# Manta-Network/manta-rs

Measured on AMD Instinct MI355X. Metric: G1 MSM Mscalar/s at 2^20, higher is better.
Workload: dtype u32; 1 GPU; 2^20 BLS12-381 G1 variable-base MSM per GPU, uniform scalars resident in HBM; curve=BLS12-381, log_n=20, window_bits=17, msms_in_flight=3

## Files before the change

### include/mantagpu.h

```cpp
#ifndef MANTAGPU_H
#define MANTAGPU_H
#include <stddef.h>
#include <stdint.h>

#ifdef __cplusplus
extern "C" {
#endif

typedef enum { MG_BN254 = 0, MG_BLS12_381 = 1 } mg_curve_t;

enum {
    MG_SUCCESS = 0,
    MG_ERROR_INVALID_ARGUMENT = 1,
    MG_ERROR_HIP = 2,
    MG_ERROR_OUT_OF_MEMORY = 3,
    MG_ERROR_DOMAIN_TOO_LARGE = 4,
    MG_ERROR_STATE = 5,
    MG_ERROR_CHECKSUM = 6
};

typedef struct mg_bases mg_bases;
typedef struct mg_msm_job mg_msm_job;
typedef struct mg_ctx mg_ctx;

int mg_init(int device);
const char *mg_strerror(int status);
const char *mg_last_error(void);
int mg_device_count(int *count);
int mg_malloc(void **dptr, size_t bytes);
int mg_free(void *dptr);
int mg_memcpy_h2d(void *dptr, const void *hptr, size_t bytes);
int mg_memcpy_d2h(void *hptr, const void *dptr, size_t bytes);
int mg_device_synchronize(void);
int mg_host_alloc(void **hptr, size_t bytes);
int mg_host_free(void *hptr);
int mg_set_kernel_timing(int on);
float mg_last_accumulate_ms(void);
float mg_last_accumulate_mhz(void);
int mg_clock_probe(unsigned iters, double *memtime_mhz, double *mad_issue_per_us_per_simd, double *ms);
int mg_last_ntt_ms(float out4[4]);
int mg_last_prove_phases_ms(float out10[10]);
int mg_last_pass_host_ms(float out3[3]);
int mg_hw_queues(int out2[2]);

int mg_bases_create(mg_curve_t curve, int group, const uint64_t *affine_mont, size_t n, int on_device,
                    int precompute_window_bits, mg_bases **out);
int mg_bases_create_sharded(mg_curve_t curve, int group, const uint64_t *affine_mont, size_t n, const int *devices,
                            int n_devices, int precompute_window_bits, mg_bases **out);
int mg_bases_num_shards(const mg_bases *bases);
int mg_bases_shard(const mg_bases *bases, int shard, int *device, size_t *lo, size_t *hi);
void mg_bases_destroy(mg_bases *bases);
size_t mg_bases_device_bytes(const mg_bases *bases);
int mg_msm(const mg_bases *bases, const uint64_t *scalars_canonical, size_t n, uint64_t *out_affine_mont);
#define MG_SCALARS_MONT 1
#define MG_SCALARS_SPARSE 2
int mg_msm_launch(const mg_bases *bases, const uint64_t *d_scalars, size_t n, int scalar_flags, int window_bits,
                  mg_msm_job **job);
int mg_msm_launch_sharded(const mg_bases *bases, const uint64_t *const *d_scalars_per_shard, int scalar_flags,
                          int window_bits, mg_msm_job **job);
int mg_msm_finish(mg_msm_job *job, uint64_t *out_affine_mont);
int mg_msm_result_to_device(mg_msm_job *job, uint64_t *d_out_xyzz, void *stream);
size_t mg_xyzz_limbs(mg_curve_t curve, int group);
int mg_xyzz_sum(mg_curve_t curve, int group, const uint64_t *xyzz, size_t n, uint64_t *out_affine_mont);
int mg_points_sum(mg_curve_t curve, int group, const uint64_t *affine_mont, size_t n, uint64_t *out_affine_mont);
int mg_fixed_base_mul(mg_curve_t curve, int group, const uint64_t *base_affine_mont, const uint64_t *d_scalars,
                      size_t n, uint64_t *d_out_affine_mont);
#define MG_EC_ADD_MIXED 0
#define MG_EC_ADD 1
#define MG_EC_DOUBLE 2
#define MG_EC_MUL 3
#define MG_EC_SUB_MIXED 4
#define MG_EC_MUL_FIXED 5
int mg_ec_elementwise(mg_curve_t curve, int group, int op, const uint64_t *a_affine, const uint64_t *b, size_t n,
                      uint64_t *out_affine);
#define MG_FIELD_ADD 0
#define MG_FIELD_SUB 1
#define MG_FIELD_MUL 2
#define MG_FIELD_SQR 3
#define MG_FIELD_NEG 4
#define MG_FIELD_FROM_CANONICAL 5
#define MG_FIELD_TO_CANONICAL 6
#define MG_FIELD_INV 7
int mg_field_op(int field, int op, int repr, int lazy_a, int lazy_b, const uint64_t *a, const uint64_t *b, size_t n,
                uint64_t *out);
int mg_msm_digits(mg_curve_t curve, const uint64_t *scalars, size_t batch, size_t n_scalars, int scalar_flags, int window_bits,
                  int table_mode, size_t n, const uint32_t *map, size_t n_sets, size_t set_len, int compact, uint32_t *keys,
                  uint32_t *vals, uint32_t *count, uint32_t layout[4]);
int mg_sort_pairs(const uint32_t *keys, const uint32_t *vals, size_t n, int end_bit, const uint32_t *count, uint32_t lowmask,
                  uint32_t inv_from, uint32_t *keys_out, uint32_t *vals_out);
int mg_group_ntt(mg_curve_t curve, int group, const uint64_t *points_affine, unsigned log_n, int inverse, uint64_t *out_affine);
int mg_point_serialize(mg_curve_t curve, int group, const uint64_t *affine_mont, int compressed, uint8_t *out);

int mg_ntt(mg_curve_t curve, uint64_t *data_mont, unsigned log_n, int inverse, int coset);
int mg_ntt_device(mg_curve_t curve, uint64_t *d_data_mont, unsigned log_n, int inverse, int coset);

typedef struct {
// ... 232 lines not shown
```

### manta_rs_amd/api.py

```python
from __future__ import annotations

import ctypes
import os

import numpy as np

_HERE = os.path.dirname(os.path.abspath(__file__))
LIB_PATH = os.environ.get("MANTA_LIB") or os.path.join(_HERE, "lib", "libmantagpu.so")

BN254, BLS12_381 = 0, 1
FQ_LIMBS = {BN254: 4, BLS12_381: 6}


class MantaGpuError(RuntimeError):

    def __init__(self, status, where=""):
        self.status = status
        detail = LIB.mg_last_error().decode() if status == 2 else ""
        super().__init__(f"{where}: {LIB.mg_strerror(status).decode()} ({status}) {detail}")


def _load():
    if not os.path.exists(LIB_PATH):
        raise ImportError(
            f"{LIB_PATH} not found: the MI355X HIP library is the product and there is no CPU fallback. "
            "Run `python -c 'import __graft_entry__ as g; g.build()'` (or `make -C manta_rs_amd/csrc`).")
    try:
        import torch
    except Exception:
        pass
    lib = ctypes.CDLL(LIB_PATH, mode=ctypes.RTLD_GLOBAL)
    lib.mg_strerror.restype = ctypes.c_char_p
    lib.mg_last_error.restype = ctypes.c_char_p
    lib.mg_bases_device_bytes.restype = ctypes.c_size_t
    lib.mg_ctx_domain_size.restype = ctypes.c_uint64
    lib.mg_ctx_num_variables.restype = ctypes.c_uint64
    lib.mg_ctx_num_inputs.restype = ctypes.c_uint64
    lib.mg_last_accumulate_ms.restype = ctypes.c_float
    lib.mg_last_accumulate_mhz.restype = ctypes.c_float
    lib.mg_vk_encoded_size.restype = ctypes.c_size_t
    lib.mg_vk_num_inputs.restype = ctypes.c_uint64
    lib.mg_xyzz_limbs.restype = ctypes.c_size_t
    lib.mg_partials_slot_limbs.restype = ctypes.c_size_t
    return lib


LIB = _load()
_vp = ctypes.c_void_p
_sz = ctypes.c_size_t

EXPORTS = [
    "mg_init", "mg_strerror", "mg_last_error", "mg_device_count", "mg_malloc", "mg_free", "mg_memcpy_h2d",
    "mg_memcpy_d2h", "mg_device_synchronize", "mg_host_alloc", "mg_host_free", "mg_set_kernel_timing", "mg_last_accumulate_ms", "mg_bases_create", "mg_bases_destroy", "mg_bases_device_bytes",
    "mg_msm", "mg_msm_launch", "mg_msm_finish", "mg_points_sum", "mg_fixed_base_mul", "mg_ec_elementwise", "mg_point_serialize", "mg_ntt",
    "mg_msm_digits", "mg_sort_pairs",
    "mg_ntt_device", "mg_groth16_setup", "mg_ctx_create", "mg_ctx_create_from_bytes", "mg_ctx_set_r1cs", "mg_groth16_prove", "mg_groth16_prove_batch", "mg_witness_map", "mg_ctx_domain_size", "mg_ctx_table_bytes",
    "mg_ctx_destroy", "mg_bases_create_sharded", "mg_bases_num_shards", "mg_bases_shard", "mg_msm_launch_sharded",
    "mg_ctx_create_sharded", "mg_ctx_create_from_bytes_sharded", "mg_ctx_num_variables", "mg_ctx_num_inputs",
    "mg_ctx_num_shards", "mg_field_op", "mg_vk_create", "mg_vk_create_from_bytes", "mg_vk_encoded_size", "mg_vk_encode",
    "mg_vk_alpha_beta", "mg_vk_num_inputs", "mg_vk_destroy", "mg_groth16_verify", "mg_groth16_verify_batch", "mg_pairing_check", "mg_proof_decode", "mg_group_ntt",
    "mg_msm_result_to_device", "mg_xyzz_limbs", "mg_xyzz_sum", "mg_ctx_create_shard", "mg_partials_slot_limbs",
    "mg_groth16_partials_launch", "mg_groth16_partials_finish", "mg_groth16_assemble", "mg_blake3", "mg_ctx_create_from_bytes_checked",
    "mg_last_ntt_ms", "mg_hw_queues", "mg_last_prove_phases_ms", "mg_clock_probe", "mg_last_accumulate_mhz", "mg_ctx_create_task",
    "mg_ctx_opts_init", "mg_ctx_create_ex", "mg_ctx_create_from_bytes_ex", "mg_last_pass_host_ms",
    "mg_tuning_init", "mg_get_tuning", "mg_set_tuning", "mg_tuning_env_names",
    "mg_points_decode", "mg_points_check", "mg_points_encode", "mg_proofs_decode",
    "mg_poseidon_create", "mg_poseidon_destroy", "mg_poseidon_permute", "mg_poseidon_hash", "mg_poseidon_hash_device",
    "mg_merkle_tree", "mg_merkle_forest_roots",
    "mg_edwards_decode", "mg_edwards_encode", "mg_edwards_check", "mg_edwards_mul", "mg_edwards_add",
    "mg_note_cipher_create", "mg_note_cipher_destroy", "mg_notes_encrypt", "mg_notes_decrypt",
    "mg_utxo_model_create", "mg_utxo_model_destroy", "mg_utxos_mint", "mg_utxos_open", "mg_viewing_keys",
    "mg_blake2s256", "mg_schnorr_challenges", "mg_signatures_verify", "mg_signatures_sign",
    "mg_blake2s", "mg_aes256_gcm", "mg_address_partitions", "mg_merkle_shard_indices",
    "mg_light_notes_encrypt", "mg_light_notes_open", "mg_outgoing_notes_encrypt", "mg_outgoing_notes_open",
]


def _chk(rc, where):
    if rc != 0:
        raise MantaGpuError(rc, where)


def _p(a):
    return None if a is None else a.ctypes.data_as(_vp)


def _u64(a):
    return np.ascontiguousarray(a, dtype=np.uint64)


def _addr(x):
    if x is None:
        return None
    if isinstance(x, ctypes.c_void_p):
        return x
    if hasattr(x, "ptr"):
        return _addr(x.ptr)
    return _vp(int(x))


def init(device=0):
    _chk(LIB.mg_init(int(device)), "mg_init")


def device_count():
    c = ctypes.c_int(0)
    _chk(LIB.mg_device_count(ctypes.byref(c)), "mg_device_count")
    return c.value


def set_kernel_timing(on):
    _chk(LIB.mg_set_kernel_timing(int(bool(on))), "mg_set_kernel_timing")


def last_accumulate_ms():
    return float(LIB.mg_last_accumulate_ms())


def last_accumulate_mhz():
    return float(LIB.mg_last_accumulate_mhz())


def clock_probe(iters=200000):
    a, b, c = ctypes.c_double(0), ctypes.c_double(0), ctypes.c_double(0)
    _chk(LIB.mg_clock_probe(ctypes.c_uint(iters), ctypes.byref(a), ctypes.byref(b), ctypes.byref(c)), "mg_clock_probe")
    return a.value, b.value, c.value


def last_ntt_ms():
    v = (ctypes.c_float * 4)()
    _chk(LIB.mg_last_ntt_ms(v), "mg_last_ntt_ms")
    return [float(x) for x in v]


def hw_queues():
    v = (ctypes.c_int * 2)()
    _chk(LIB.mg_hw_queues(v), "mg_hw_queues")
    return int(v[0]), int(v[1])


def last_prove_phases_ms():
    v = (ctypes.c_float * 10)()
    _chk(LIB.mg_last_prove_phases_ms(v), "mg_last_prove_phases_ms")
    names = ("upload_z", "witness_map", "msm_a", "msm_b_g1", "msm_b_g2", "msm_l", "msm_h", "part_a_upload_to_join", "g2_chain_upload_to_end",
             "host_assembly_after_gpu")
    return {n: round(float(x), 4) for n, x in zip(names, v)}


def last_pass_host_ms():
    v = (ctypes.c_float * 3)()
    _chk(LIB.mg_last_pass_host_ms(v), "mg_last_pass_host_ms")
    return {"enqueue": round(float(v[0]), 4), "wait_gpu": round(float(v[1]), 4), "assemble": round(float(v[2]), 4)}


def synchronize():
    _chk(LIB.mg_device_synchronize(), "mg_device_synchronize")


class PinnedArray:

    def __init__(self, shape, dtype=np.uint64):
        self.nbytes = int(np.prod(shape)) * np.dtype(dtype).itemsize
        ptr = _vp()
        _chk(LIB.mg_host_alloc(ctypes.byref(ptr), _sz(self.nbytes)), "mg_host_alloc")
        self._ptr = ptr
        buf = (ctypes.c_uint8 * self.nbytes).from_address(ptr.value)
        self.array = np.frombuffer(buf, dtype=dtype).reshape(shape)

    @classmethod
    def like(cls, arr):
        arr = np.ascontiguousarray(arr)
        p = cls(arr.shape, arr.dtype)
        p.array[...] = arr
        return p

    def free(self):
        if self._ptr is not None and self._ptr.value:
            self.array = None
            LIB.mg_host_free(self._ptr)
            self._ptr = None

    def __del__(self):
        try:
            self.free()
        except Exception:
            pass


class DeviceBuffer:

    def __init__(self, nbytes):
# ... 1099 lines not shown
```

### manta_rs_amd/csrc/capi.cpp

```cpp
#include "../../include/mantagpu.h"
#include "engine.h"
#include "staging.h"
#include "tuning.h"
#include <cstddef>
#include "prover.h"
#include "verify.h"
#include "edwards.h"
#include "utxo.h"
#include "schnorr.h"
#include "light_note.h"
#include <cstring>
#include <new>
#include <vector>

using namespace mg;

struct BasesShard {
    GroupEngine *eng;
    BaseSet *bs;
    int device;
    size_t lo, hi;
};
struct mg_bases {
    std::vector<BasesShard> sh;
// ... 46 lines not shown
    return MG_SUCCESS;
}
MG_API int mg_free(void *dptr) {
    MG_HIP(hipFree(dptr));
    return MG_SUCCESS;
}
MG_API int mg_host_alloc(void **hptr, size_t bytes) {
    if (!hptr) return MG_ERROR_INVALID_ARGUMENT;
    MG_HIP(hipHostMalloc(hptr, bytes ? bytes : 1, hipHostMallocDefault));
    return MG_SUCCESS;
}
MG_API int mg_host_free(void *hptr) {
    MG_HIP(hipHostFree(hptr));
    return MG_SUCCESS;
}
MG_API int mg_memcpy_h2d(void *d, const void *h, size_t bytes) {
    MG_HIP(memcpy_sync(d, h, bytes, hipMemcpyHostToDevice));
    return MG_SUCCESS;
}
MG_API int mg_memcpy_d2h(void *h, const void *d, size_t bytes) {
    MG_HIP(memcpy_sync(h, d, bytes, hipMemcpyDeviceToHost));
    return MG_SUCCESS;
}
MG_API int mg_device_synchronize(void) {
    MG_HIP(hipDeviceSynchronize());
    return MG_SUCCESS;
}

MG_API int mg_set_kernel_timing(int on) {
    set_kernel_timing(on != 0);
    return MG_SUCCESS;
}
MG_API float mg_last_accumulate_ms(void) { return last_accumulate_ms(); }
MG_API float mg_last_accumulate_mhz(void) { return last_accumulate_mhz(); }
namespace mg {
int clock_probe(u32 iters, double *memtime_mhz, double *mad_issue_per_us_per_simd, double *ms);
}
MG_API int mg_clock_probe(unsigned iters, double *memtime_mhz, double *mad_issue_per_us_per_simd, double *ms) {
    MG_TRY
    if (iters == 0 || iters > (1u << 24)) return MG_ERROR_INVALID_ARGUMENT;
    return clock_probe(iters, memtime_mhz, mad_issue_per_us_per_simd, ms);
    MG_CATCH
}
MG_API int mg_last_ntt_ms(float out4[4]) {
    if (!out4) return MG_ERROR_INVALID_ARGUMENT;
    get_last_ntt_ms(out4);
    return MG_SUCCESS;
}
MG_API int mg_hw_queues(int out2[2]) {
    if (!out2) return MG_ERROR_INVALID_ARGUMENT;
    out2[0] = out2[1] = 0;
    (void)stream_queue_counts(&out2[0], &out2[1]);
    return MG_SUCCESS;
}
MG_API int mg_last_pass_host_ms(float out3[3]) {
    if (!out3) return MG_ERROR_INVALID_ARGUMENT;
    get_last_pass_host_ms(out3);
    return MG_SUCCESS;
}
MG_API int mg_last_prove_phases_ms(float out10[10]) {
    if (!out10) return MG_ERROR_INVALID_ARGUMENT;
    get_last_prove_ms(out10);
    return MG_SUCCESS;
}

static void bases_free(mg_bases *b) {
    DeviceGuard guard;
    for (BasesShard &s : b->sh) {
        hipSetDevice(s.device);
        if (s.bs) s.eng->bases_destroy(s.bs);
    }
    delete b;
}
static int bases_create_on(mg_curve_t curve, int group, const uint64_t *affine, size_t n, int on_device, int pre_c,
                           const int *devices, int n_devices, mg_bases **out) {
    if (!out || !affine || n == 0 || pre_c < -12 || pre_c == -1 || pre_c > 24 || n_devices < 1 || n_devices > 64 || (size_t)n_devices > n)
        return MG_ERROR_INVALID_ARGUMENT;
    if (on_device && n_devices != 1) return MG_ERROR_INVALID_ARGUMENT;
    int count = 0;
    MG_HIP(hipGetDeviceCount(&count));
    DeviceGuard guard;
    mg_bases *b = new mg_bases();
    b->n = n;
    for (int g = 0; g < n_devices; ++g) {
        const int dev = devices ? devices[g] : guard.prev;
        if (dev < 0 || dev >= count || dev >= MAX_DEVICES) {
            bases_free(b);
            return MG_ERROR_INVALID_ARGUMENT;
        }
        hipError_t he = hipSetDevice(dev);
        GroupEngine *e = he == hipSuccess ? get_engine((int)curve, group) : nullptr;
        if (!e) {
            bases_free(b);
            return he == hipSuccess ? MG_ERROR_INVALID_ARGUMENT : MG_ERROR_HIP;
        }
        const size_t lo = n * (size_t)g / n_devices, hi = n * (size_t)(g + 1) / n_devices;
        BaseSet *bs = nullptr;
        int rc = e->bases_create((const u32 *)affine + lo * (size_t)e->affine_words(), hi - lo, on_device != 0, pre_c, &bs);
        if (rc) {
            bases_free(b);
            return rc;
        }
        b->sh.push_back(BasesShard{e, bs, dev, lo, hi});
    }
    *out = b;
    return MG_SUCCESS;
// ... 895 lines not shown
```

### manta_rs_amd/csrc/ec_dev.h

```cpp
#pragma once
#include "fp_dev.h"

namespace mg {

#define MG_EC_CALL __device__ __noinline__

template <class F, int B> struct Bv {
    F v;
};
template <int B, class F> MG_DEV Bv<F, B> bv(const F &f) { return Bv<F, B>{f}; }
template <class F, int A, int B> MG_DEV Bv<F, F::BM> operator*(const Bv<F, A> &a, const Bv<F, B> &b) {
    static_assert((long)A * B * F::MULK <= F::LIM, "product of operand bounds exceeds the Montgomery headroom");
    return Bv<F, F::BM>{F::template mulb<A, B>(a.v, b.v)};
}
template <class F, int A> MG_DEV Bv<F, F::BM> b_sqr(const Bv<F, A> &a) {
    static_assert((long)A * A * F::MULK <= F::LIM, "square of operand bound exceeds the Montgomery headroom");
    return Bv<F, F::BM>{F::template sqrb<A>(a.v)};
}
template <class F, int A, int B> MG_DEV Bv<F, A + B> operator+(const Bv<F, A> &a, const Bv<F, B> &b) {
    return Bv<F, A + B>{F::add(a.v, b.v)};
}
template <class F, int A> MG_DEV Bv<F, 2 * A> b_dbl(const Bv<F, A> &a) { return Bv<F, 2 * A>{F::dbl(a.v)}; }
template <class F, int A, int B> MG_DEV Bv<F, A + B> operator-(const Bv<F, A> &a, const Bv<F, B> &b) {
    static_assert(B <= F::MAXM, "no multiple of p large enough for this subtrahend");
// ... 74 lines not shown
        auto X2 = b_sqr(px);
        auto M = b_fit<6>(b_dbl(X2) + X2);
        auto X3 = b_fit<BX>(b_sub2(b_sqr(M), bv<0>(F::zero()), S));
        auto Y3 = b_fit<BY>(M * (S - X3) - W * py);
        X3o = X3.v;
        Y3o = Y3.v;
        Vo = V.v;
        Wo = W.v;
    }
    static MG_EC_CALL XYZZ dbl_affine_call(const Affine<F> &p) { return dbl_affine_body(p); }
    static MG_DEV XYZZ dbl_affine(const Affine<F> &p) {
        if constexpr (F::EXT) return dbl_affine_call(p);
        else return dbl_affine_body(p);
    }
    static MG_DEV XYZZ dbl_affine_body(const Affine<F> &p) {
        XYZZ r;
        dbl_core(bv<BM>(p.x), bv<BM>(p.y), r.x, r.y, r.zz, r.zzz);
        return r;
    }
    static MG_EC_CALL XYZZ dbl_call(const XYZZ &p) { return dbl_body(p); }
    static MG_DEV XYZZ dbl(const XYZZ &p) {
        if constexpr (F::EXT) return dbl_call(p);
        else return dbl_body(p);
    }
    static MG_DEV XYZZ dbl_body(const XYZZ &p) {
        if (p.is_inf()) return p;
        XYZZ r;
        F V, W;
        dbl_core(bv<BX>(p.x), bv<BY>(p.y), r.x, r.y, V, W);
        r.zz = (bv<BM>(V) * bv<BM>(p.zz)).v;
        r.zzz = (bv<BM>(W) * bv<BM>(p.zzz)).v;
        return r;
    }
    MG_EC_CALL void madd_call(const Affine<F> &q, bool neg) { madd_body(q, neg); }
    MG_DEV void madd(const Affine<F> &q, bool neg) {
        if constexpr (F::EXT) madd_call(q, neg);
        else madd_body(q, neg);
    }
#ifdef MG_ACC_TWO_CHAINS
    static constexpr bool THROUGHPUT_CH = false;
#else
    static constexpr bool THROUGHPUT_CH = true;
#endif
    MG_DEV void madd_throughput(const Affine<F> &q, bool neg) {
        if constexpr (!F::EXT && F::LAZY) {
            madd_lazy<THROUGHPUT_CH>(q, neg);
            return;
        }
        madd(q, neg);
    }
    struct MaddCarry {
        F P, R, PP;
    };
    template <bool CH = false> MG_DEV bool madd_begin(const Affine<F> &q_in, bool negate, MaddCarry &c) {
        static_assert(!F::EXT && F::LAZY, "reduced-radix base field only");
        static_assert(F::BX == 8 && F::BY == 4 && F::BM == 2 && F::LIM >= 121, "bound analysis above");
        constexpr bool LL = F::LAZY_LIMBS;
        if (q_in.is_inf()) return false;
        F qy = q_in.y;
        if (negate) {
            if constexpr (LL) qy = F::template negl<3>(q_in.y);
            else qy = F::template neg<2>(q_in.y);
        }
        if (is_inf()) {
            x = q_in.x;
            y = negate ? F::template neg<2>(q_in.y) : q_in.y;
            zz = F::one();
            zzz = F::one();
            return false;
        }
        const F U2 = F::template mul_t<CH>(q_in.x, zz);
        const F S2 = F::template mul_t<CH>(qy, zzz);
        if constexpr (LL) {
            c.P = F::template subl<9>(U2, x);
            c.R = F::template subl<5>(S2, y);
        } else {
            c.P = F::template sub<8>(U2, x);
            c.R = F::template sub<4>(S2, y);
        }
        c.PP = F::template sqr_t<CH>(c.P);
        if (c.PP.template is_zero_mod<2>()) {
            if ((LL ? F::normalize_u(c.R) : c.R).template is_zero_mod<7>()) {
                Affine<F> q{q_in.x, negate ? F::template neg<2>(q_in.y) : q_in.y};
                *this = dbl_affine(q);
            } else {
                *this = inf();
            }
            return false;
        }
        return true;
    }
    template <bool CH = false> MG_DEV void madd_finish(const MaddCarry &c) {
        constexpr bool LL = F::LAZY_LIMBS;
        const F PPP = F::template mul_t<CH>(c.P, c.PP);
        const F Q = F::template mul_t<CH>(x, c.PP);
        const F X3 = F::template sub2<6>(F::template sqr_t<CH>(c.R), PPP, Q);
        F T, N;
        if constexpr (LL) {
            T = F::template subl<9>(Q, X3);
            N = F::template negl<3>(PPP);
        } else {
            T = F::template sub<8>(Q, X3);
            N = F::template neg<2>(PPP);
        }
        const F Y3 = F::template mul_add_t<CH>(c.R, T, y, N);
        zz = F::template mul_t<CH>(zz, c.PP);
        zzz = F::template mul_t<CH>(zzz, PPP);
        x = X3;
        y = Y3;
    }
    template <bool CH = false> MG_DEV void madd_lazy(const Affine<F> &q_in, bool negate) {
        MaddCarry c;
        if (madd_begin<CH>(q_in, negate, c)) madd_finish<CH>(c);
    }
    MG_DEV void madd_body(const Affine<F> &q_in, bool negate) {
        if constexpr (!F::EXT && F::LAZY) {
            madd_lazy<false>(q_in, negate);
            return;
        }
        if (q_in.is_inf()) return;
        Affine<F> q = q_in;
        if (negate) q.y = b_neg(bv<BM>(q.y)).v;
        if (is_inf()) {
            x = q.x;
            y = q.y;
            zz = F::one();
            zzz = F::one();
            return;
        }
        const auto X1 = bv<BX>(x);
        const auto Y1 = bv<BY>(y);
        const auto ZZ1 = bv<BM>(zz);
        const auto ZZZ1 = bv<BM>(zzz);
        auto U2 = bv<BM>(q.x) * ZZ1;
        auto S2 = bv<BM>(q.y) * ZZZ1;
        auto P = U2 - X1;
        auto R = S2 - Y1;
        if (b_is_zero(P)) {
            if (b_is_zero(R))
                *this = dbl_affine(q);
            else
                *this = inf();
            return;
        }
        auto PP = b_sqr(P);
        auto PPP = P * PP;
// ... 103 lines not shown
```

### manta_rs_amd/csrc/engine.h

```cpp
#pragma once
#include <hip/hip_runtime.h>
#include <shared_mutex>
#include <atomic>
#include <cstddef>
#include <cstdint>
#include <mutex>
#include <vector>

namespace mg {

typedef uint32_t u32;
typedef uint64_t u64;

#ifdef MG_NO_PRIO
#define MG_PRIO_HIGH() ((void)0)
#else
#define MG_PRIO_HIGH() __builtin_amdgcn_s_setprio(3)
#endif
#define MG_PRIO_FOR(F) MG_PRIO_HIGH()

enum { MG_OK = 0, MG_ERR_ARG = 1, MG_ERR_HIP = 2, MG_ERR_OOM = 3, MG_ERR_DOMAIN = 4, MG_ERR_STATE = 5 };

void set_last_hip_error(hipError_t e, const char *expr, const char *file, int line);
inline int hip_status(hipError_t e, const char *what, const char *file = __builtin_FILE(), int line = __builtin_LINE()) {
// ... 44 lines not shown
void stream_pool_put_normal(hipStream_t s);
struct GraphClient {
    GraphClient();
    ~GraphClient();
    GraphClient(const GraphClient &) = delete;
    GraphClient &operator=(const GraphClient &) = delete;
};
int graph_clients_alive();
hipStream_t stream_pool_get_dedicated();
void stream_pool_put_dedicated(hipStream_t s);
struct StreamSet {
    hipStream_t main = nullptr, g2 = nullptr, z3 = nullptr;
    int id = -1, dev = 0;
    bool z3_high = false;
};
bool stream_sets_ready();
int stream_queue_counts(int *normal, int *high);
bool stream_set_acquire(StreamSet &s, bool z3_high);
void stream_set_release(StreamSet &s);
int streams_share_queue(hipStream_t a, hipStream_t b, unsigned *mem, unsigned *token_counter);
const char *last_error_string();

struct DeviceScope {
    int prev = 0;
    bool switched = false;
    explicit DeviceScope(int dev) {
        if (hipGetDevice(&prev) == hipSuccess && prev != dev) switched = hipSetDevice(dev) == hipSuccess;
    }
    ~DeviceScope() {
        if (switched) hipSetDevice(prev);
    }
    DeviceScope(const DeviceScope &) = delete;
    DeviceScope &operator=(const DeviceScope &) = delete;
};

struct DeviceGuard {
    int prev = 0;
    DeviceGuard() { hipGetDevice(&prev); }
    ~DeviceGuard() { hipSetDevice(prev); }
    DeviceGuard(const DeviceGuard &) = delete;
    DeviceGuard &operator=(const DeviceGuard &) = delete;
};

struct DevBuf {
    void *p = nullptr;
    size_t cap = 0;
    int reserve(size_t bytes);
    void release();
    template <class T> T *as() const { return (T *)p; }
};

enum { SCALARS_CANONICAL = 0, SCALARS_MONT = 1, SCALARS_WORK = 2 };

struct MsmPlan {
    int c = 0;
    int W = 0;
    u32 B = 0;
    int Wb = 0;
    bool precomp = false;
    bool full = false;
    u32 L = 0;
};

struct BaseSet {
    int curve = 0, group = 1;
    int device = 0;
    size_t n = 0;
    size_t n_orig = 0;
    u32 *d_map = nullptr;
    u32 *d_pts = nullptr;
    int pre_c = 0, pre_W = 0;
    bool full = false;
    u32 n_sets = 1;
    size_t set_len = 0;
    static constexpr u32 MAX_SETS = 4;
    u32 set_first[MAX_SETS + 1] = {};
    size_t bytes = 0;
};

enum MsmTailKind : u32 { TAIL_WINDOW_SUMS = 0, TAIL_X_SUMS = 1, TAIL_TWO_LEVELS = 2 };
struct MsmTail {
    static constexpr int MAX_EXTRA = 8;
    MsmTailKind kind = TAIL_WINDOW_SUMS;
    u32 T1 = 0, nP = 0, segs = 0;
    u32 tail_shift = 0, n_extra = 0, extra_shift[MAX_EXTRA] = {};
    size_t extra_off_pts = 0;
    const u32 *d_tail = nullptr;
};

struct MsmWorkspace {
    DevBuf keys_in, keys_out, vals_in, vals_out, sort_tmp, buckets, pkeys[2], ppts[2], redA, redS, misc;
    DevBuf count;
    DevBuf front, extra;
    DevBuf folded;
    unsigned long long *h_clk = nullptr;
    DevBuf scratch;
    void *h_stage = nullptr;
    size_t h_stage_cap = 0;
    hipStream_t stream = nullptr;
    hipStream_t run_on = nullptr;
    hipStream_t solo = nullptr;
    bool use_solo = false;
    hipStream_t side_stream = nullptr;
    hipEvent_t side_fork = nullptr, side_join = nullptr;
    hipEvent_t done = nullptr;
    hipEvent_t t0 = nullptr, t1 = nullptr;
// ... 110 lines not shown
```

### manta_rs_amd/csrc/msm_accumulate.h

```cpp
#pragma once
#include "msm_common.h"

namespace mg {

#ifndef MG_ACC_INPLACE
#define MG_ACC_INPLACE 1
#endif
#ifndef MG_ACC_BLOCK
#define MG_ACC_BLOCK 0
#endif
#ifndef MG_ACC_AHEAD
#define MG_ACC_AHEAD 0
#endif
#ifndef MG_ACC_SINGLE_ROTATED
#define MG_ACC_SINGLE_ROTATED 0
#endif
template <class F> struct AccChunksRotated : std::false_type {};
template <> struct AccChunksRotated<FpR<Bls381FqCfg>> : std::integral_constant<bool, MG_ACC_INPLACE != 0> {};
template <class F> constexpr bool acc_chunks_rotated() { return AccChunksRotated<F>::value; }
#ifdef MG_ACC_WAVES
#define MG_ACC_ATTR __attribute__((amdgpu_waves_per_eu(MG_ACC_WAVES, MG_ACC_WAVES)))
#else
#define MG_ACC_ATTR
#endif
template <class F, bool PROBE = false>
__global__ __launch_bounds__(256) MG_ACC_ATTR void accumulate_chunks(const u32 *__restrict__ keys, const u32 *__restrict__ vals,
                                                         u32 M, u32 L, u32 invalid, const u32 *__restrict__ bases,
                                                         u32 astride, u32 *__restrict__ buckets,
                                                         u32 *__restrict__ pkeys, u32 *__restrict__ ppts, u32 T,
                                                         const u32 *__restrict__ count, unsigned long long *__restrict__ clk,
                                                         u32 adapt) {
    const u32 t = blockIdx.x * blockDim.x + threadIdx.x;
    if (t >= T) return;
    long long c0 = 0;
    unsigned long long w0 = 0;
    if constexpr (PROBE)
        if (t == 0) c0 = clock64(), w0 = wall_clock64();
    if (count) {
        M = *count;
        if (adapt) {
            const u32 l = (M + T - 1) / T;
            L = l > L ? l : L;
        }
    }
    const size_t begin = (size_t)t * L;
    size_t end = begin + L;
    if (end > M) end = M;
    u32 cur = begin < M ? keys[begin] : invalid;
    if (cur == invalid) {
        pkeys[2 * t] = invalid;
        pkeys[2 * t + 1] = invalid;
        return;
    }
    XYZZ<F> acc = XYZZ<F>::inf();
    bool first = true;
    auto close_run = [&]() {
        if (first) {
            pkeys[2 * t] = cur;
            acc.store(ppts + (size_t)(2 * t) * XYZZ<F>::WORDS);
            first = false;
        } else {
            acc.store(buckets + (size_t)cur * XYZZ<F>::WORDS);
        }
        acc = XYZZ<F>::inf();
    };
    if constexpr (acc_chunks_rotated<F>()) {
        u32 kn = invalid, vn = 0;
        [[maybe_unused]] uint4 kb, vb;
        auto load_block = [&](size_t i) {
            if (i + 4 <= end) {
                kb = *reinterpret_cast<const uint4 *>(keys + i);
                vb = *reinterpret_cast<const uint4 *>(vals + i);
            }
        };
        auto next_pair = [&](size_t i) {
            if constexpr (MG_ACC_BLOCK) {
                const u32 q = (u32)i & 3u;
                if (i - q >= begin && i - q + 4 <= end) {
                    if (q == 0) load_block(i);
                    kn = q == 0 ? kb.x : (q == 1 ? kb.y : (q == 2 ? kb.z : kb.w));
                    vn = q == 0 ? vb.x : (q == 1 ? vb.y : (q == 2 ? vb.z : vb.w));
                    return;
                }
            }
            kn = keys[i], vn = vals[i];
        };
        size_t j = begin;
        u32 k = cur, v = vals[j];
        Affine<F> p = Affine<F>::load(bases + (size_t)(v & 0x7fffffffu) * astride);
        if constexpr (MG_ACC_BLOCK)
            if ((begin & 3) == 0) load_block(begin);
        if (j + 1 < end) next_pair(j + 1);
        bool more;
        do {
            if (k != cur) {
                close_run();
                cur = k;
            }
            typename XYZZ<F>::MaddCarry c;
            const bool general = acc.template madd_begin<XYZZ<F>::THROUGHPUT_CH>(p, (v >> 31) != 0, c);
            auto fetch = [&]() {
                ++j;
                more = j < end && kn != invalid;
                k = kn;
                v = vn;
                if (more) {
                    p = Affine<F>::load(bases + (size_t)(v & 0x7fffffffu) * astride);
                    if (j + 1 < end) next_pair(j + 1);
                }
            };
            if constexpr (MG_ACC_AHEAD) fetch();
            if (general) acc.template madd_finish<XYZZ<F>::THROUGHPUT_CH>(c);
            if constexpr (!MG_ACC_AHEAD) fetch();
        } while (more);
        if (j < end) {
            close_run();
            cur = invalid;
        }
    } else {
        for (size_t j = begin; j < end; ++j) {
            const u32 k = keys[j];
            if (k != cur) {
                close_run();
                cur = k;
                if (k == invalid) break;
            }
            const u32 v = vals[j];
            const Affine<F> p = Affine<F>::load(bases + (size_t)(v & 0x7fffffffu) * astride);
            acc.madd_throughput(p, (v >> 31) != 0);
        }
    }
    if (first) {
        pkeys[2 * t] = cur;
        acc.store(ppts + (size_t)(2 * t) * XYZZ<F>::WORDS);
        pkeys[2 * t + 1] = cur;
        XYZZ<F>::inf().store(ppts + (size_t)(2 * t + 1) * XYZZ<F>::WORDS);
    } else {
        pkeys[2 * t + 1] = cur;
        acc.store(ppts + (size_t)(2 * t + 1) * XYZZ<F>::WORDS);
    }
    if constexpr (PROBE)
        if (t == 0) clk[0] = (unsigned long long)(clock64() - c0), clk[1] = wall_clock64() - w0;
}

template <class F> struct AccSingle {
    static constexpr int XW = XYZZ<F>::WORDS;
    static constexpr int PAIR = F::EXT ? 1 : 0;
    static constexpr int SLOTS = 256 >> PAIR, PER = SLOTS / 64;
    typedef CoopAdd<F, false> Coop;
    static constexpr size_t LDS_BYTES = ((size_t)SLOTS * XW + Coop::LDS_WORDS) * 4;
};
template <class F>
__global__ __launch_bounds__(256) MG_TAIL_ATTR void accumulate_single(const u32 *__restrict__ vals, u32 M, u32 L, const u32 *__restrict__ bases,
                                                                      u32 astride, u32 *__restrict__ pkeys, u32 *__restrict__ ppts, u32 T,
                                                                      const u32 *__restrict__ count, u32 adapt, u32 invalid) {
    extern __shared__ __attribute__((aligned(16))) u32 acc_single_lds[];
    constexpr int XW = AccSingle<F>::XW, PAIR = AccSingle<F>::PAIR, SLOTS = AccSingle<F>::SLOTS, PER = AccSingle<F>::PER;
    u32 *xs = acc_single_lds;
    u32 *cx = acc_single_lds + SLOTS * XW;
    const u32 t = blockIdx.x * blockDim.x + threadIdx.x;
    const int lane = threadIdx.x & 63, wave = threadIdx.x >> 6;
    if (count) {
        M = *count;
        if (adapt) {
            const u32 l = (M + T - 1) / T;
            L = l > L ? l : L;
        }
    }
    XYZZ<F> acc = XYZZ<F>::inf();
    const size_t begin = (size_t)t * L;
    size_t end = begin + L;
    if (end > M) end = M;
    if constexpr (MG_ACC_SINGLE_ROTATED && MG_ACC_INPLACE && !F::EXT && F::LAZY) {
        if (t < T && begin < end) {
            size_t j = begin;
            u32 v = vals[j], vn = 0;
            Affine<F> p = Affine<F>::load(bases + (size_t)(v & 0x7fffffffu) * astride);
            if (j + 1 < end) vn = vals[j + 1];
            bool more;
            do {
                typename XYZZ<F>::MaddCarry c;
                const bool general = acc.template madd_begin<XYZZ<F>::THROUGHPUT_CH>(p, (v >> 31) != 0, c);
                auto fetch = [&]() {
                    ++j;
                    more = j < end;
                    v = vn;
                    if (more) {
                        p = Affine<F>::load(bases + (size_t)(v & 0x7fffffffu) * astride);
                        if (j + 1 < end) vn = vals[j + 1];
                    }
                };
                if constexpr (MG_ACC_AHEAD) fetch();
                if (general) acc.template madd_finish<XYZZ<F>::THROUGHPUT_CH>(c);
                if constexpr (!MG_ACC_AHEAD) fetch();
            } while (more);
        }
// ... 58 lines not shown
```

### manta_rs_amd/csrc/msm_bls381_g1.hip

```cpp
#include "msm_impl.h"
namespace mg {
GroupEngine *make_engine_bls381_g1() { return new GroupEngineT<Bls381, 1, 1>(); }
}
```

### manta_rs_amd/csrc/msm_engine.h

```cpp
#pragma once
#include "msm_common.h"
#include "staging.h"
#include "msm_digits.h"
#include "msm_accumulate.h"
#include "msm_reduce.h"
#include "msm_tables.h"

namespace mg {

template <class Curve, int GROUP> struct GT;
template <class Curve> struct GT<Curve, 1> {
#ifdef MG_G1_SATURATED
    typedef Fp<typename Curve::Fq> F;
#else
    typedef FpR<typename Curve::Fq> F;
#endif
    typedef Fp<typename Curve::Fq> FIO;
    typedef host::HFp<typename Curve::Fq> HF;
};
template <class Curve> struct GT<Curve, 2> {
#ifdef MG_G2_SATURATED
    typedef Fp2<typename Curve::Fq> F;
#else
    typedef Fp2R<typename Curve::Fq> F;
// ... 216 lines not shown
    }
    int expand_full_tables(const u32 *win_pts, u32 *final_pts, size_t n, int W, u32 FB) {
        const size_t pairs = (size_t)W * n;
        size_t slice = ((size_t)512 << 20) / ((size_t)FB * XW * 4);
        if (slice < 256) slice = 256;
        if (slice > pairs) slice = pairs;
        u32 *tmp = nullptr;
        hipError_t e = hipMalloc((void **)&tmp, slice * FB * XW * 4);
        constexpr int KBF = 64;
        for (size_t j0 = 0; e == hipSuccess && j0 < pairs; j0 += slice) {
            const size_t cntp = pairs - j0 < slice ? pairs - j0 : slice;
            hipLaunchKernelGGL((full_table_chain<F>), dim3(cdiv(cntp, 256)), dim3(256), 0, setup_stream(), win_pts, (u32)AWS, j0, (u32)cntp, FB,
                               tmp);
            hipLaunchKernelGGL((xyzz_to_affine_batch<F, KBF>), dim3(cdiv(cdiv(cntp * FB, KBF), 256)), dim3(256), 0, setup_stream(), tmp,
                               cntp * FB, final_pts + j0 * FB * AWS, (u32)AWS);
            e = hipGetLastError();
        }
        if (e == hipSuccess) e = setup_sync();
        else (void)setup_sync();
        if (tmp) hipFree(tmp);
        return e == hipSuccess ? MG_OK : hip_status(e, "full-table kernels");
    }
    void bases_destroy(BaseSet *bs) override {
        if (!bs) return;
        if (bs->d_map) hipFree(bs->d_map);
        if (bs->d_pts) hipFree(bs->d_pts);
        delete bs;
    }

    MsmPlan plan_for(const BaseSet *bs, size_t n, int c_override, u32 batch = 1) const override {
        MsmPlan p;
        if (bs->pre_c > 0) {
            p.c = bs->pre_c;
            p.W = bs->pre_W;
            p.precomp = true;
            p.full = bs->full;
            p.Wb = 1;
        } else {
            int lg = 0;
            while (((size_t)1 << lg) < n) ++lg;
            int c = c_override > 0 ? c_override : (lg <= 8 ? 5 : lg <= 12 ? 8 : lg <= 15 ? 10 : lg <= 18 ? 12 : lg <= 19 ? 14 : 16);
            p.c = c;
            p.W = windows_of(c);
            p.Wb = p.W;
        }
        p.B = 1u << (p.c - 1);
        const size_t M = n * (size_t)p.W * batch;
        size_t L;
        if (M < ((size_t)8 << 20)) {
            L = M / (192 * 1024);
            if (L < 6) L = 6;
            if (p.full) L = 3;
        } else {
            const size_t round = 128 * 1024, lmax = batch > 1 ? 96 : 192;
            const size_t rounds = (M + round * lmax - 1) / (round * lmax);
            L = (M + round * rounds - 1) / (round * rounds);
        }
        if (msm_knobs().msm_L > 0) L = (size_t)msm_knobs().msm_L;
        p.L = (u32)L;
        return p;
    }

    u32 acc_round_lanes(bool batched, bool single = false) {
        const int knob = msm_knobs().acc_round_waves;
        if (knob == 0) return 0;
        const int dev = current_device();
        if (dev < 0 || dev >= 64 || !occ_[dev].cus.load(std::memory_order_acquire)) return 0;
        u32 w = single && occ_[dev].blocks_single ? occ_[dev].blocks_single : occ_[dev].blocks;
        if (knob > 0) w = (u32)knob < w ? (u32)knob : w;
        else if (batched && w > 2) w = 2;
        return w * 256u * occ_[dev].cus.load(std::memory_order_relaxed);
    }
    struct Occ {
        u32 blocks = 0, blocks_single = 0;
        std::atomic<u32> cus{0};
    } occ_[64];
    void prime_occupancy() {
        const int dev = current_device();
        if (dev < 0 || dev >= 64 || occ_[dev].cus.load(std::memory_order_acquire)) return;
        int nb = 0, cus = 0;
        if (hipOccupancyMaxActiveBlocksPerMultiprocessor(&nb, accumulate_chunks<F, false>, 256, 0) != hipSuccess ||
            hipDeviceGetAttribute(&cus, hipDeviceAttributeMultiprocessorCount, dev) != hipSuccess || nb < 1 || cus < 1) {
            (void)hipGetLastError();
            return;
        }
        int nbs = 0;
        if (hipFuncSetAttribute(reinterpret_cast<const void *>(&accumulate_single<F>), hipFuncAttributeMaxDynamicSharedMemorySize,
                                (int)AccSingle<F>::LDS_BYTES) != hipSuccess ||
            hipOccupancyMaxActiveBlocksPerMultiprocessor(&nbs, accumulate_single<F>, 256, AccSingle<F>::LDS_BYTES) != hipSuccess || nbs < 1) {
            (void)hipGetLastError();
            nbs = 0;
        }
        std::lock_guard<std::mutex> g(side_mu_);
        occ_[dev].blocks_single = (u32)nbs;
        occ_[dev].blocks = (u32)nb;
        occ_[dev].cus.store((u32)cus, std::memory_order_release);
    }

    static bool coop_tiles(u32 tiles) { return (int)tiles <= msm_knobs().coop_tiles; }
    static u32 merge_g1(size_t M) {
        if (const u32 g = msm_knobs().merge_g) return g;
        return M < ((size_t)8 << 20) ? 16u : 4u;
    }

    static void tile_reduce_launch(hipStream_t st, u32 items, bool may_coop, const u32 *in, u32 stride, u32 off, u32 n, u32 tiles,
                                   u32 *A, u32 *S, int std_out) {
        if (may_coop && coop_tiles(items))
            hipLaunchKernelGGL((tile_reduce_coop<F>), dim3(items), dim3(256), 0, st, in, stride, off, n, tiles, A, S, std_out);
        else
            hipLaunchKernelGGL((tile_reduce<F>), dim3(cdiv(items, 4)), dim3(256), 0, st, in, stride, off, n, tiles, items, A, S, std_out);
    }
    static void serial_reduce_launch(hipStream_t st, size_t lanes_all, const u32 *in, u32 stride, u32 off, u32 n, u32 S, u32 lanes,
                                     u32 *A, u32 *Sx) {
        if (cdiv(lanes_all, 64) <= msm_knobs().coop_waves)
            hipLaunchKernelGGL((serial_reduce_coop<F>), dim3(cdiv(lanes_all, 64)), dim3(256), 0, st, in, stride, off, n, S, lanes,
                               (u32)lanes_all, A, Sx);
// ... 656 lines not shown
```

### rust/mantagpu-sys/src/lib.rs

```rust
#![no_std]
#![allow(non_camel_case_types)]

use core::ffi::{c_char, c_float, c_int, c_uint, c_void};

pub type mg_curve_t = c_int;
pub const MG_BN254: mg_curve_t = 0;
pub const MG_BLS12_381: mg_curve_t = 1;

pub const MG_SUCCESS: c_int = 0;
pub const MG_ERROR_INVALID_ARGUMENT: c_int = 1;
pub const MG_ERROR_HIP: c_int = 2;
pub const MG_ERROR_OUT_OF_MEMORY: c_int = 3;
pub const MG_ERROR_DOMAIN_TOO_LARGE: c_int = 4;
pub const MG_ERROR_STATE: c_int = 5;
pub const MG_ERROR_CHECKSUM: c_int = 6;
pub const MG_TASK_A: c_uint = 1;
pub const MG_TASK_B_G1: c_uint = 2;
pub const MG_TASK_B_G2: c_uint = 4;
pub const MG_TASK_L: c_uint = 8;
pub const MG_TASK_H: c_uint = 16;

pub const MG_SCALARS_MONT: c_int = 1;
pub const MG_SCALARS_SPARSE: c_int = 2;

// ... 133 lines not shown
    pub full_table_bytes: i64,
    pub devices: *const c_int,
    pub n_devices: i32,
    pub shard: i32,
    pub n_shards: i32,
    pub task_mask: u32,
    pub tuning: *const mg_tuning,
}
pub const MG_EXCHANGE_HOST: u32 = 0;
pub const MG_EXCHANGE_RCCL: u32 = 1;

#[repr(C)]
pub struct mg_csr {
    pub row_ptr: *const u32,
    pub col: *const u32,
    pub val: *const u64,
    pub nnz: u64,
}

#[repr(C)]
pub struct mg_pk_out {
    pub alpha_g1: *mut u64,
    pub beta_g1: *mut u64,
    pub delta_g1: *mut u64,
    pub beta_g2: *mut u64,
    pub gamma_g2: *mut u64,
    pub delta_g2: *mut u64,
    pub gamma_abc_g1: *mut u64,
    pub a_query: *mut u64,
    pub b_g1_query: *mut u64,
    pub b_g2_query: *mut u64,
    pub h_query: *mut u64,
    pub l_query: *mut u64,
}

extern "C" {
    pub fn mg_init(device: c_int) -> c_int;
    pub fn mg_strerror(status: c_int) -> *const c_char;
    pub fn mg_last_error() -> *const c_char;
    pub fn mg_device_count(count: *mut c_int) -> c_int;
    pub fn mg_malloc(dptr: *mut *mut c_void, bytes: usize) -> c_int;
    pub fn mg_free(dptr: *mut c_void) -> c_int;
    pub fn mg_memcpy_h2d(dptr: *mut c_void, hptr: *const c_void, bytes: usize) -> c_int;
    pub fn mg_memcpy_d2h(hptr: *mut c_void, dptr: *const c_void, bytes: usize) -> c_int;
    pub fn mg_device_synchronize() -> c_int;
    pub fn mg_host_alloc(hptr: *mut *mut c_void, bytes: usize) -> c_int;
    pub fn mg_host_free(hptr: *mut c_void) -> c_int;
    pub fn mg_set_kernel_timing(on: c_int) -> c_int;
    pub fn mg_last_accumulate_ms() -> c_float;
    pub fn mg_last_accumulate_mhz() -> c_float;
    pub fn mg_clock_probe(iters: c_uint, memtime_mhz: *mut f64, mad_issue_per_us_per_simd: *mut f64, ms: *mut f64) -> c_int;
    pub fn mg_last_ntt_ms(out4: *mut c_float) -> c_int;
    pub fn mg_hw_queues(out2: *mut c_int) -> c_int;
    pub fn mg_last_prove_phases_ms(out10: *mut c_float) -> c_int;
    pub fn mg_last_pass_host_ms(out3: *mut c_float) -> c_int;

    pub fn mg_bases_create(
        curve: mg_curve_t,
        group: c_int,
        affine_mont: *const u64,
        n: usize,
        on_device: c_int,
        precompute_window_bits: c_int,
        out: *mut *mut mg_bases,
    ) -> c_int;
    pub fn mg_bases_create_sharded(
        curve: mg_curve_t,
        group: c_int,
        affine_mont: *const u64,
        n: usize,
        devices: *const c_int,
        n_devices: c_int,
        precompute_window_bits: c_int,
        out: *mut *mut mg_bases,
    ) -> c_int;
    pub fn mg_bases_num_shards(bases: *const mg_bases) -> c_int;
    pub fn mg_bases_shard(bases: *const mg_bases, shard: c_int, device: *mut c_int, lo: *mut usize, hi: *mut usize) -> c_int;
    pub fn mg_bases_destroy(bases: *mut mg_bases);
    pub fn mg_bases_device_bytes(bases: *const mg_bases) -> usize;
    pub fn mg_msm(bases: *const mg_bases, scalars_canonical: *const u64, n: usize, out_affine_mont: *mut u64) -> c_int;
    pub fn mg_msm_launch(
        bases: *const mg_bases,
        d_scalars: *const u64,
        n: usize,
        scalar_flags: c_int,
        window_bits: c_int,
        job: *mut *mut mg_msm_job,
    ) -> c_int;
    pub fn mg_msm_launch_sharded(
        bases: *const mg_bases,
        d_scalars_per_shard: *const *const u64,
        scalar_flags: c_int,
        window_bits: c_int,
        job: *mut *mut mg_msm_job,
    ) -> c_int;
    pub fn mg_msm_finish(job: *mut mg_msm_job, out_affine_mont: *mut u64) -> c_int;
    pub fn mg_msm_result_to_device(job: *mut mg_msm_job, d_out_xyzz: *mut u64, stream: *mut c_void) -> c_int;
    pub fn mg_xyzz_limbs(curve: mg_curve_t, group: c_int) -> usize;
    pub fn mg_xyzz_sum(curve: mg_curve_t, group: c_int, xyzz: *const u64, n: usize, out_affine_mont: *mut u64) -> c_int;
    pub fn mg_points_sum(curve: mg_curve_t, group: c_int, affine_mont: *const u64, n: usize, out_affine_mont: *mut u64) -> c_int;
    pub fn mg_fixed_base_mul(
        curve: mg_curve_t,
        group: c_int,
        base_affine_mont: *const u64,
        d_scalars: *const u64,
        n: usize,
// ... 410 lines not shown
```

Before: 421.5 Mscalar/s.

## Size MSM chunk length from occupancy lanes and add lean accumulate variant

Chunk length for large MSMs is now computed from the actual resident lane count (CUs × occupancy blocks × 256) instead of a fixed 128K-lane round, so rounds match the hardware's concurrent threads. A compile-time lean accumulate variant is added: it uses 32-bit indices, defers the doubling case out of madd_begin, and schedules madd_finish with sched barriers to cut register pressure, with waves-per-EU set to 3. The BLS12-381 accumulate kernel moves into its own compilation unit so it can take these flags, but MG_ACC_LEAN defaults to 0, so only the chunk-length change runs by default.

Result: no change. 421.3 Mscalar/s, median of 2 (-0.1%).

```diff
diff --git a/include/mantagpu.h b/include/mantagpu.h
--- a/include/mantagpu.h
+++ b/include/mantagpu.h
@@ -42,6 +42,7 @@
 int mg_last_prove_phases_ms(float out10[10]);
 int mg_last_pass_host_ms(float out3[3]);
 int mg_hw_queues(int out2[2]);
+uint32_t mg_msm_large_chunk_length(uint64_t pairs, uint32_t round_lanes, int batched);
 
 int mg_bases_create(mg_curve_t curve, int group, const uint64_t *affine_mont, size_t n, int on_device,
                     int precompute_window_bits, mg_bases **out);
diff --git a/manta_rs_amd/api.py b/manta_rs_amd/api.py
--- a/manta_rs_amd/api.py
+++ b/manta_rs_amd/api.py
@@ -37,6 +37,8 @@
     lib.mg_ctx_num_variables.restype = ctypes.c_uint64
     lib.mg_ctx_num_inputs.restype = ctypes.c_uint64
     lib.mg_last_accumulate_ms.restype = ctypes.c_float
+    lib.mg_msm_large_chunk_length.restype = ctypes.c_uint32
+    lib.mg_msm_large_chunk_length.argtypes = [ctypes.c_uint64, ctypes.c_uint32, ctypes.c_int]
     lib.mg_last_accumulate_mhz.restype = ctypes.c_float
     lib.mg_vk_encoded_size.restype = ctypes.c_size_t
     lib.mg_vk_num_inputs.restype = ctypes.c_uint64
@@ -61,7 +63,7 @@
     "mg_vk_alpha_beta", "mg_vk_num_inputs", "mg_vk_destroy", "mg_groth16_verify", "mg_groth16_verify_batch", "mg_pairing_check", "mg_proof_decode", "mg_group_ntt",
     "mg_msm_result_to_device", "mg_xyzz_limbs", "mg_xyzz_sum", "mg_ctx_create_shard", "mg_partials_slot_limbs",
     "mg_groth16_partials_launch", "mg_groth16_partials_finish", "mg_groth16_assemble", "mg_blake3", "mg_ctx_create_from_bytes_checked",
-    "mg_last_ntt_ms", "mg_hw_queues", "mg_last_prove_phases_ms", "mg_clock_probe", "mg_last_accumulate_mhz", "mg_ctx_create_task",
+    "mg_last_ntt_ms", "mg_hw_queues", "mg_msm_large_chunk_length", "mg_last_prove_phases_ms", "mg_clock_probe", "mg_last_accumulate_mhz", "mg_ctx_create_task",
     "mg_ctx_opts_init", "mg_ctx_create_ex", "mg_ctx_create_from_bytes_ex", "mg_last_pass_host_ms",
     "mg_tuning_init", "mg_get_tuning", "mg_set_tuning", "mg_tuning_env_names",
     "mg_points_decode", "mg_points_check", "mg_points_encode", "mg_proofs_decode",
@@ -137,6 +139,10 @@
     v = (ctypes.c_int * 2)()
     _chk(LIB.mg_hw_queues(v), "mg_hw_queues")
     return int(v[0]), int(v[1])
+
+
+def msm_large_chunk_length(pairs, round_lanes, batched=False):
+    return int(LIB.mg_msm_large_chunk_length(int(pairs), int(round_lanes), int(bool(batched))))
 
 
 def last_prove_phases_ms():
diff --git a/manta_rs_amd/csrc/capi.cpp b/manta_rs_amd/csrc/capi.cpp
--- a/manta_rs_amd/csrc/capi.cpp
+++ b/manta_rs_amd/csrc/capi.cpp
@@ -122,6 +122,9 @@
     out2[0] = out2[1] = 0;
     (void)stream_queue_counts(&out2[0], &out2[1]);
     return MG_SUCCESS;
+}
+MG_API uint32_t mg_msm_large_chunk_length(uint64_t pairs, uint32_t round_lanes, int batched) {
+    return round_lanes ? msm_large_chunk_length((size_t)pairs, round_lanes, batched != 0) : 0u;
 }
 MG_API int mg_last_pass_host_ms(float out3[3]) {
     if (!out3) return MG_ERROR_INVALID_ARGUMENT;
diff --git a/manta_rs_amd/csrc/ec_dev.h b/manta_rs_amd/csrc/ec_dev.h
--- a/manta_rs_amd/csrc/ec_dev.h
+++ b/manta_rs_amd/csrc/ec_dev.h
@@ -150,11 +150,16 @@
     struct MaddCarry {
         F P, R, PP;
     };
-    template <bool CH = false> MG_DEV bool madd_begin(const Affine<F> &q_in, bool negate, MaddCarry &c) {
+    enum { MADD_DONE = 0, MADD_GENERAL = 1, MADD_DOUBLE = 2 };
+    MG_DEV void madd_double(const Affine<F> &q_in, bool negate) {
+        Affine<F> q{q_in.x, negate ? F::template neg<2>(q_in.y) : q_in.y};
+        *this = dbl_affine(q);
+    }
+    template <bool CH = false, bool DEFER = false> MG_DEV int madd_begin(const Affine<F> &q_in, bool negate, MaddCarry &c) {
         static_assert(!F::EXT && F::LAZY, "reduced-radix base field only");
         static_assert(F::BX == 8 && F::BY == 4 && F::BM == 2 && F::LIM >= 121, "bound analysis above");
         constexpr bool LL = F::LAZY_LIMBS;
-        if (q_in.is_inf()) return false;
+        if (q_in.is_inf()) return MADD_DONE;
         F qy = q_in.y;
         if (negate) {
             if constexpr (LL) qy = F::template negl<3>(q_in.y);
@@ -165,7 +170,7 @@
             y = negate ? F::template neg<2>(q_in.y) : q_in.y;
             zz = F::one();
             zzz = F::one();
-            return false;
+            return MADD_DONE;
         }
         const F U2 = F::template mul_t<CH>(q_in.x, zz);
         const F S2 = F::template mul_t<CH>(qy, zzz);
@@ -179,17 +184,42 @@
         c.PP = F::template sqr_t<CH>(c.P);
         if (c.PP.template is_zero_mod<2>()) {
             if ((LL ? F::normalize_u(c.R) : c.R).template is_zero_mod<7>()) {
-                Affine<F> q{q_in.x, negate ? F::template neg<2>(q_in.y) : q_in.y};
-                *this = dbl_affine(q);
+                if constexpr (DEFER) return MADD_DOUBLE;
+                madd_double(q_in, negate);
             } else {
                 *this = inf();
             }
-            return false;
-        }
-        return true;
-    }
-    template <bool CH = false> MG_DEV void madd_finish(const MaddCarry &c) {
+            return MADD_DONE;
+        }
+        return MADD_GENERAL;
+    }
+    template <bool CH = false, bool ORDERED = false> MG_DEV void madd_finish(const MaddCarry &c) {
         constexpr bool LL = F::LAZY_LIMBS;
+        if constexpr (ORDERED) {
+            const F PPP = F::template mul_t<CH>(c.P, c.PP);
+            __builtin_amdgcn_sched_barrier(0);
+            const F Q = F::template mul_t<CH>(x, c.PP);
+            __builtin_amdgcn_sched_barrier(0);
+            zz = F::template mul_t<CH>(zz, c.PP);
+            __builtin_amdgcn_sched_barrier(0);
+            zzz = F::template mul_t<CH>(zzz, PPP);
+            __builtin_amdgcn_sched_barrier(0);
+            const F RR = F::template sqr_t<CH>(c.R);
+            __builtin_amdgcn_sched_barrier(0);
+            x = F::template sub2<6>(RR, PPP, Q);
+            F T, N;
+            if constexpr (LL) {
+                T = F::template subl<9>(Q, x);
+                N = F::template negl<3>(PPP);
+            } else {
+                T = F::template sub<8>(Q, x);
+                N = F::template neg<2>(PPP);
+            }
+            __builtin_amdgcn_sched_barrier(0);
+            y = F::template mul_add_t<CH>(c.R, T, y, N);
+            __builtin_amdgcn_sched_barrier(0);
+            return;
+        }
         const F PPP = F::template mul_t<CH>(c.P, c.PP);
         const F Q = F::template mul_t<CH>(x, c.PP);
         const F X3 = F::template sub2<6>(F::template sqr_t<CH>(c.R), PPP, Q);
diff --git a/manta_rs_amd/csrc/engine.h b/manta_rs_amd/csrc/engine.h
--- a/manta_rs_amd/csrc/engine.h
+++ b/manta_rs_amd/csrc/engine.h
@@ -120,6 +120,11 @@
 
 enum { SCALARS_CANONICAL = 0, SCALARS_MONT = 1, SCALARS_WORK = 2 };
 
+inline u32 msm_large_chunk_length(size_t M, size_t round, bool batched) {
+    const size_t lmax = batched ? 96 : 192;
+    const size_t rounds = (M + round * lmax - 1) / (round * lmax);
+    return (u32)((M + round * rounds - 1) / (round * rounds));
+}
 struct MsmPlan {
     int c = 0;
     int W = 0;
diff --git a/manta_rs_amd/csrc/msm_accumulate.h b/manta_rs_amd/csrc/msm_accumulate.h
--- a/manta_rs_amd/csrc/msm_accumulate.h
+++ b/manta_rs_amd/csrc/msm_accumulate.h
@@ -14,10 +14,14 @@
 #endif
 #ifndef MG_ACC_SINGLE_ROTATED
 #define MG_ACC_SINGLE_ROTATED 0
+#endif
+#ifndef MG_ACC_LEAN
+#define MG_ACC_LEAN 0
 #endif
 template <class F> struct AccChunksRotated : std::false_type {};
 template <> struct AccChunksRotated<FpR<Bls381FqCfg>> : std::integral_constant<bool, MG_ACC_INPLACE != 0> {};
 template <class F> constexpr bool acc_chunks_rotated() { return AccChunksRotated<F>::value; }
+template <class F> constexpr bool acc_chunks_lean() { return acc_chunks_rotated<F>() && MG_ACC_LEAN != 0 && !MG_ACC_BLOCK && !MG_ACC_AHEAD; }
 #ifdef MG_ACC_WAVES
 #define MG_ACC_ATTR __attribute__((amdgpu_waves_per_eu(MG_ACC_WAVES, MG_ACC_WAVES)))
 #else
@@ -32,10 +36,14 @@
                                                          u32 adapt) {
     const u32 t = blockIdx.x * blockDim.x + threadIdx.x;
     if (t >= T) return;
+    constexpr bool LEAN = acc_chunks_lean<F>();
     long long c0 = 0;
     unsigned long long w0 = 0;
     if constexpr (PROBE)
-        if (t == 0) c0 = clock64(), w0 = wall_clock64();
+        if (t == 0) {
+            c0 = clock64(), w0 = wall_clock64();
+            if constexpr (LEAN) clk[2] = (unsigned long long)c0, clk[3] = w0;
+        }
     if (count) {
         M = *count;
         if (adapt) {
@@ -73,7 +81,8 @@
                 vb = *reinterpret_cast<const uint4 *>(vals + i);
             }
         };
-        auto next_pair = [&](size_t i) {
+        typedef typename std::conditional<LEAN, u32, size_t>::type idx_t;
+        auto next_pair = [&](idx_t i) {
             if constexpr (MG_ACC_BLOCK) {
                 const u32 q = (u32)i & 3u;
                 if (i - q >= begin && i - q + 4 <= end) {
@@ -85,12 +94,13 @@
             }
             kn = keys[i], vn = vals[i];
         };
-        size_t j = begin;
+        idx_t j = (idx_t)begin;
+        const idx_t jend = (idx_t)end;
         u32 k = cur, v = vals[j];
         Affine<F> p = Affine<F>::load(bases + (size_t)(v & 0x7fffffffu) * astride);
         if constexpr (MG_ACC_BLOCK)
             if ((begin & 3) == 0) load_block(begin);
-        if (j + 1 < end) next_pair(j + 1);
+        if (j + 1 < jend) next_pair(j + 1);
         bool more;
         do {
             if (k != cur) {
@@ -98,22 +108,25 @@
                 cur = k;
             }
             typename XYZZ<F>::MaddCarry c;
-            const bool general = acc.template madd_begin<XYZZ<F>::THROUGHPUT_CH>(p, (v >> 31) != 0, c);
+            const int step = acc.template madd_begin<XYZZ<F>::THROUGHPUT_CH, LEAN>(p, (v >> 31) != 0, c);
             auto fetch = [&]() {
                 ++j;
-                more = j < end && kn != invalid;
+                more = j < jend && kn != invalid;
                 k = kn;
                 v = vn;
                 if (more) {
                     p = Affine<F>::load(bases + (size_t)(v & 0x7fffffffu) * astride);
-                    if (j + 1 < end) next_pair(j + 1);
+                    if (j + 1 < jend) next_pair(j + 1);
                 }
             };
             if constexpr (MG_ACC_AHEAD) fetch();
-            if (general) acc.template madd_finish<XYZZ<F>::THROUGHPUT_CH>(c);
+            if (step == XYZZ<F>::MADD_GENERAL) acc.template madd_finish<XYZZ<F>::THROUGHPUT_CH, LEAN>(c);
+            if constexpr (LEAN)
+                if (step == XYZZ<F>::MADD_DOUBLE)
+                    acc.madd_double(Affine<F>::load(bases + (size_t)(v & 0x7fffffffu) * astride), (v >> 31) != 0);
             if constexpr (!MG_ACC_AHEAD) fetch();
         } while (more);
-        if (j < end) {
+        if (j < jend) {
             close_run();
             cur = invalid;
         }
@@ -140,8 +153,19 @@
         acc.store(ppts + (size_t)(2 * t + 1) * XYZZ<F>::WORDS);
     }
     if constexpr (PROBE)
-        if (t == 0) clk[0] = (unsigned long long)(clock64() - c0), clk[1] = wall_clock64() - w0;
-}
+        if (t == 0) {
+            const long long c1 = clock64();
+            const unsigned long long w1 = wall_clock64();
+            if constexpr (LEAN) c0 = (long long)clk[2], w0 = clk[3];
+            clk[0] = (unsigned long long)(c1 - c0), clk[1] = w1 - w0;
+        }
+}
+
+#define MG_ACC_CHUNKS_UNIT(KW, F)                                                                                                   \
+    KW template __global__ void accumulate_chunks<F, false>(const u32 *, const u32 *, u32, u32, u32, const u32 *, u32, u32 *, u32 *, \
+                                                            u32 *, u32, const u32 *, unsigned long long *, u32);                     \
+    KW template __global__ void accumulate_chunks<F, true>(const u32 *, const u32 *, u32, u32, u32, const u32 *, u32, u32 *, u32 *,  \
+                                                           u32 *, u32, const u32 *, unsigned long long *, u32);
 
 template <class F> struct AccSingle {
     static constexpr int XW = XYZZ<F>::WORDS;
diff --git a/manta_rs_amd/csrc/msm_bls381_g1.hip b/manta_rs_amd/csrc/msm_bls381_g1.hip
--- a/manta_rs_amd/csrc/msm_bls381_g1.hip
+++ b/manta_rs_amd/csrc/msm_bls381_g1.hip
@@ -1,3 +1,7 @@
+#include "msm_accumulate.h"
+namespace mg {
+MG_ACC_CHUNKS_UNIT(extern, FpR<Bls381FqCfg>)
+}
 #include "msm_impl.h"
 namespace mg {
 GroupEngine *make_engine_bls381_g1() { return new GroupEngineT<Bls381, 1, 1>(); }
diff --git a/manta_rs_amd/csrc/msm_bls381_g1_acc.hip b/manta_rs_amd/csrc/msm_bls381_g1_acc.hip
--- /dev/null
+++ b/manta_rs_amd/csrc/msm_bls381_g1_acc.hip
@@ -0,0 +1,10 @@
+#ifndef MG_ACC_LEAN
+#define MG_ACC_LEAN 0
+#endif
+#if MG_ACC_LEAN && !defined(MG_ACC_WAVES)
+#define MG_ACC_WAVES 3
+#endif
+#include "msm_accumulate.h"
+namespace mg {
+MG_ACC_CHUNKS_UNIT(, FpR<Bls381FqCfg>)
+}
diff --git a/manta_rs_amd/csrc/msm_engine.h b/manta_rs_amd/csrc/msm_engine.h
--- a/manta_rs_amd/csrc/msm_engine.h
+++ b/manta_rs_amd/csrc/msm_engine.h
@@ -292,16 +292,15 @@
             if (L < 6) L = 6;
             if (p.full) L = 3;
         } else {
-            const size_t round = 128 * 1024, lmax = batch > 1 ? 96 : 192;
-            const size_t rounds = (M + round * lmax - 1) / (round * lmax);
-            L = (M + round * rounds - 1) / (round * rounds);
+            const u32 lanes = acc_round_lanes(batch > 1);
+            L = msm_large_chunk_length(M, lanes ? lanes : 128 * 1024, batch > 1);
         }
         if (msm_knobs().msm_L > 0) L = (size_t)msm_knobs().msm_L;
         p.L = (u32)L;
         return p;
     }
 
-    u32 acc_round_lanes(bool batched, bool single = false) {
+    u32 acc_round_lanes(bool batched, bool single = false) const {
         const int knob = msm_knobs().acc_round_waves;
         if (knob == 0) return 0;
         const int dev = current_device();
diff --git a/rust/mantagpu-sys/src/lib.rs b/rust/mantagpu-sys/src/lib.rs
--- a/rust/mantagpu-sys/src/lib.rs
+++ b/rust/mantagpu-sys/src/lib.rs
@@ -209,6 +209,7 @@
     pub fn mg_clock_probe(iters: c_uint, memtime_mhz: *mut f64, mad_issue_per_us_per_simd: *mut f64, ms: *mut f64) -> c_int;
     pub fn mg_last_ntt_ms(out4: *mut c_float) -> c_int;
     pub fn mg_hw_queues(out2: *mut c_int) -> c_int;
+    pub fn mg_msm_large_chunk_length(pairs: u64, round_lanes: u32, batched: c_int) -> u32;
     pub fn mg_last_prove_phases_ms(out10: *mut c_float) -> c_int;
     pub fn mg_last_pass_host_ms(out3: *mut c_float) -> c_int;
 
```
